# selftok-team/SelftokTokenizer

Hardware: AMD Instinct MI355X
Metric: images/sec encode+decode, 256x256 512-token (higher is better)
Workload: dtype f32

## Files before the change

include/selftok_hip.h:

```cpp
#ifndef SELFTOK_HIP_H
#define SELFTOK_HIP_H

#include <stddef.h>
#include <stdint.h>

#ifdef __cplusplus
extern "C" {
#endif

#ifndef __HIP__
typedef struct ihipStream_t* hipStream_t;
#endif

#define SELFTOK_OK 0
#define SELFTOK_EINVAL (-1)
#define SELFTOK_EHIP (-2)

#define SELFTOK_IDS_I32 1
#define SELFTOK_PRENORMED 2
#define SELFTOK_VQ_F16COARSE 8
#define SELFTOK_VQ_F16COARSE1 16
#define SELFTOK_VQ_RT(n) (((n) & 0xF) << 8)
#define SELFTOK_VQ_SPLIT(n) (((n) & 0xFF) << 16)

int selftok_version(void);
const char* selftok_last_error(void);

size_t selftok_vq_workspace_bytes(int N, int C);
int selftok_vq_encode_f32(const float* z, const float* codebook, void* ids, float* best, void* workspace,
                          int N, int C, int D, int flags, hipStream_t stream);
size_t selftok_vq_packed_bytes(int C, int D);
int selftok_vq_pack_codebook(const float* codebook, float* packed, int C, int D, hipStream_t stream);
int selftok_vq_encode_packed_f32(const float* z, const float* packed, void* ids, float* best, void* workspace,
                                 int N, int C, int D, int flags, hipStream_t stream);

int selftok_vq_argmax_partial_packed_f32(const float* z, const float* packed, void* workspace, int* nsplit_out,
                                         int N, int C, int D, int flags, hipStream_t stream);
int selftok_vq_finalize_packed(const void* workspace, const float* z, const float* packed, void* ids, float* best,
                               int N, int C, int D, int nsplit, int flags, hipStream_t stream);

int selftok_code_gather_ln_f32(const void* ids, const float* codebook, const float* ln_w, const float* ln_b,
                               float* out, int n, int C, int D, float eps, int flags, hipStream_t stream);

int selftok_vq_ema_accumulate_f32(const float* z, const void* ids, float* bins, float* embed_sum, int N, int C, int D, int flags, hipStream_t stream);
int selftok_vq_tpc_update_f32(float* tpc, const void* ids, int B, int K, int C, float weight, int flags, hipStream_t stream);
size_t selftok_vq_softmax_workspace_bytes(int N);
int selftok_vq_softmax_stats_f32(const float* z, const float* codebook, float* rowstats, float* colmean, void* workspace, int B, int K, int C, int D,
                                 float scale, int flags, hipStream_t stream);
int selftok_vq_softmax_backward_f32(const float* z, const float* codebook, const float* rowstats, const float* g_colmean, float* grad_z, void* workspace,
                                    int B, int K, int C, int D, float scale, int flags, hipStream_t stream);

int selftok_residual_ln_mod_f32(const float* x, const float* y, const float* gate, const float* shift, const float* scale,
                                float* x_out, float* n_out, int B, int T, int H,
                                long mod_stride_b, long mod_stride_t, long gate_stride_b, long gate_stride_t,
                                float eps, hipStream_t stream);
int selftok_residual_ln_mod_split(const float* x, const float* y, const float* gate, const float* shift, const float* scale,
                                  float* x_out, void* n_blk, int* overflow, int B, int T, int H,
                                  long mod_stride_b, long mod_stride_t, long gate_stride_b, long gate_stride_t,
                                  float eps, hipStream_t stream);

int selftok_bias_gelu_f32(float* h, const float* bias, long rows, int cols, hipStream_t stream);
int selftok_silu_f32(const float* in, float* out, long n, hipStream_t stream);
int selftok_add_rows_f32(const float* in, const float* table, float* out, int B, long per_sample, hipStream_t stream);
int selftok_timestep_embed_f32(const float* t, const float* freqs, float* out, int n, int dim, float t_scale, hipStream_t stream);
int selftok_patchify_f32(const float* x, float* out, int B, int C, int H, int W, hipStream_t stream);
int selftok_unpatchify_cfg_euler_f32(const float* y_cond, const float* y_uncond, const float* x, float* x_out, float* v_out,
                                     int B, int C, int hp, int wp, float dt, float cfg_scale, hipStream_t stream);
int selftok_rmsnorm_f32(const float* x, const float* w, float* out, long rows, int dim, float eps, hipStream_t stream);
int selftok_rotary_f32(const float* t, const float* freqs, float* out, long rows, int seq, int dim, float scale, hipStream_t stream);

#define SELFTOK_LINEAR_GELU 1
size_t selftok_linear_f16x2_packed_bytes(int N, int K);
int selftok_linear_f16x2_pack_weight(const float* W, void* packed, int N, int K, int* overflow, hipStream_t stream);
int selftok_linear_f16x2_f32(const float* A, long lda, const void* packed, const float* bias, float* out, long ldo,
                             int M, int N, int K, int flags, int* overflow, hipStream_t stream);
size_t selftok_split_f16x2_bytes(long rows, int cols);
int selftok_split_f16x2_f32(const float* x, long ld, void* blk, long rows, int cols, int* overflow, hipStream_t stream);
int selftok_linear_f16x2_split(const void* a_blk, const void* packed, const float* bias, float* out, void* out_blk, long ldo,
                               int M, int N, int K, int flags, int* overflow, hipStream_t stream);
int selftok_linear_f16x2_split_residual(const void* a_blk, const void* packed, const float* bias,
                                        const float* resid, long ldr, const float* gate, long gate_stride_b, long gate_stride_t, int T,
                                        float* out, long ldo, int M, int N, int K, int* overflow, hipStream_t stream);
size_t selftok_linear_f16x2_splitk_workspace_bytes(int M, int N, int ksplit);
int selftok_linear_f16x2_split_k(const void* a_blk, const void* packed, const float* bias, float* out, void* out_blk, long ldo,
                                 int M, int N, int K, int flags, int ksplit, void* workspace, int* overflow, hipStream_t stream);
int selftok_linear_f16x2_split_residual_k(const void* a_blk, const void* packed, const float* bias,
                                          const float* resid, long ldr, const float* gate, long gate_stride_b, long gate_stride_t, int T,
                                          float* out, long ldo, int M, int N, int K, int ksplit, void* workspace, int* overflow, hipStream_t stream);

#define SELFTOK_ATTN_F16X2 1
typedef struct selftok_attn_seg {
    const float* q; const float* k; const float* v; float* o;
    int len;
    long q_rs, k_rs, v_rs, o_rs;
    long q_bs, k_bs, v_bs, o_bs;
} selftok_attn_seg;
typedef struct selftok_attn_desc {
    selftok_attn_seg seg[2];
    int B, H, head_dim;
    const int* kvis;
    int seg0_sees_seg1;
    float scale;
    int mode;
    int* overflow;
    void* o_blk[2];
} selftok_attn_desc;
int selftok_attn_f32(const selftok_attn_desc* desc, hipStream_t stream);

int selftok_groupnorm_silu_bf16(const void* x, const void* weight, const void* bias, void* out, int B, int C, int HW, int groups,
                                float eps, int apply_silu, hipStream_t stream);
int selftok_latent_process_in(const void* moments_bf16, float* out, int B, int c_in, int c_keep, int HW, float shift, float scale, hipStream_t stream);
int selftok_latent_process_out(const float* z, void* out_bf16, long n, float shift, float scale, hipStream_t stream);
int selftok_clamp01_bf16(void* img, long n, hipStream_t stream);

size_t selftok_conv2d_packed_bytes(int Cout, int Cin, int ksize, int bn);
int selftok_conv2d_pack_weight_bf16(const void* w, void* packed, int Cout, int Cin, int ksize, int bn, hipStream_t stream);
int selftok_conv2d_nhwc_bf16(const void* x, const void* packed, const void* bias, const void* residual, void* out, int B, int H, int W, int Cin, int Cout,
                             int Cstore, int ldo, int ksize, int stride, int upsample, int bn, hipStream_t stream);
size_t selftok_groupnorm_nhwc_workspace_bytes(int B, int HW, int C);
int selftok_groupnorm_silu_nhwc_bf16(const void* x, const void* weight, const void* bias, void* out, void* workspace, int B, int HW, int C, int groups,
                                     float eps, int apply_silu, hipStream_t stream);

#define SELFTOK_VX_UPSAMPLE2X 8
int selftok_vx_conv2d_bf16(const void* x, const void* w, const void* bias, const void* residual, void* out, int B, int H, int W, int ldx, int Cin, int Cout,
                           int ksize, int stride, int order, hipStream_t stream);
size_t selftok_vx_groupnorm_workspace_bytes(int B, int HW, int C);
int selftok_vx_groupnorm_bf16(const void* x, const void* gamma, const void* beta, void* out, void* workspace, const void* silu_table, float* stats, int B, int HW,
                              int C, int groups, double eps, hipStream_t stream);
int selftok_vx_silu_table_bf16(void* table, hipStream_t stream);
size_t selftok_vx_attention_workspace_bytes(int B, int T, int C);
int selftok_vx_attention_bf16(const void* q, const void* k, const void* v, void* out, void* workspace, int B, int T, int C, hipStream_t stream);
int selftok_vx_expf_f32(const float* x, float* y, long n, hipStream_t stream);

#define SELFTOK_LINEAR_BIAS_LAST 2
#define SELFTOK_LINEAR_MKL_ORDER 4
#define SELFTOK_LINEAR_SPLIT(n) (((n) & 0xFF) << 8)
size_t selftok_linear_f32_workspace_bytes(long M, int N, int K, int flags);
int selftok_linear_f32(const float* x, long ldx, const float* w, const float* bias, const float* res, long ldr, int res_mod, const float* gate, long ldg,
                       int gate_mod, float* out, long ldo, long M, int N, int K, int flags, void* workspace, size_t workspace_bytes, hipStream_t stream);

#define SELFTOK_EX_GELU 1
#define SELFTOK_EX_BIAS_LAST 2
int selftok_ex_linear_f32(const float* x, long ldx, const float* w, const float* bias, const float* res, long ldr, int res_mod, const float* gate,
                          long ldg, int gate_mod, float* out, long ldo, long M, int N, int K, int gelu, hipStream_t stream);
int selftok_ex_layernorm_mod_f32(const float* x, long ldx, float* out, long ldo, const float* shift, const float* scale, long ldt, int T, const float* gamma,
                                 const float* beta, float* stats, long rows, int N, float eps, hipStream_t stream);
int selftok_ex_res_layernorm_mod_f32(const float* x, long ldx, const float* lin, long ldl, const float* lin_bias, const float* gate, long ldg, int gate_mod,
                                     float* x_out, long ldxo, float* out, long ldo, const float* shift, const float* scale, long ldt, int T, long rows, int N, float eps,
                                     hipStream_t stream);
int selftok_ex_unary_f32(const float* x, float* y, long n, int mode, hipStream_t stream);
size_t selftok_ex_attention_workspace_bytes(int B, int H, int Tq, int Tk, int D);
int selftok_ex_attention_f32(const float* q, long qs, const float* k1, const float* v1, long kvs1, int Tk1, int valid1, int rows1, const float* k2, const float* v2,
                             long kvs2, int Tk2, float* out, void* workspace, int B, int H, int Tq, int D, hipStream_t stream);
int selftok_ex_attention_fused_supported(int Tk1, int Tk2, int D);
int selftok_ex_attention_fused_f32(const float* q, long qs, const float* k1, const float* v1, long kvs1, int Tk1, int valid1, int rows1, const float* k2, const float* v2,
                                   long kvs2, int Tk2, float* out, int B, int H, int Tq, int D, hipStream_t stream);

#ifdef __cplusplus
}
#endif
#endif
```

selftoktokenizer_amd/csrc/attention.hip:

```cpp
#include "common.h"
#include "selftok_hip.h"
#include <stdlib.h>
#include <type_traits>

namespace selftok {

typedef float f32x16 __attribute__((ext_vector_type(16)));

struct AttnSeg {
    const float* q;
    const float* k;
    const float* v;
    float* o;
    _Float16* o_blk;
    int len;
    long q_rs, k_rs, v_rs, o_rs;
    long q_bs, k_bs, v_bs, o_bs;
};

struct AttnParams {
    AttnSeg seg[2];
    int B, H;
    const int* kvis;
    int seg0_sees_seg1;
    float scale;
    int qtiles;
    int xcd_remap;
    int prio;
};

constexpr int KT = 32;
constexpr int KSTR = 68;
constexpr int QROWS = 128;

__global__ __launch_bounds__(256) void attn64_kernel(AttnParams P)
{
    __shared__ __attribute__((aligned(16))) float s_kb[2][KT * KSTR];
    __shared__ __attribute__((aligned(16))) float s_vb[2][KT * 64];

    const int tid = threadIdx.x, lane = tid & 63, wave = tid >> 6;
    const int half = lane >> 5, col = lane & 31;
    int qt, h, b;
    {
        const int T = gridDim.x, orig = blockIdx.x;
        const int q8 = T >> 3, r8 = T & 7, xcd = orig & 7, idx = orig >> 3;
        const int w = P.xcd_remap ? (xcd < r8 ? xcd * (q8 + 1) : r8 * (q8 + 1) + (xcd - r8) * q8) + idx : orig;
        qt = w % P.qtiles;
        h = (w / P.qtiles) % P.H;
        b = w / (P.qtiles * P.H);
    }

    int n0 = P.seg[0].len;
    if (P.kvis) { int kv = P.kvis[b] + 1; n0 = kv < n0 ? (kv < 0 ? 0 : kv) : n0; }
    const int rows0 = P.seg[0].q ? n0 : 0;
    int s, r0;
    {
        const int t0 = P.seg[0].q ? (P.seg[0].len + QROWS - 1) / QROWS : 0;
        if (qt < t0) { s = 0; r0 = qt * QROWS; }
        else { s = 1; r0 = (qt - t0) * QROWS; }
    }
    const int rows_live = (s == 0) ? rows0 : (P.seg[1].q ? P.seg[1].len : 0);
    if (r0 >= rows_live) return;

    const AttnSeg& qs = P.seg[s];
    const int n1 = (s == 1 || P.seg0_sees_seg1) ? P.seg[1].len : 0;

    const int my_row = r0 + wave * 32 + col;
    const bool row_ok = my_row < rows_live;
    float qf[32];
    {
        const float* qp = qs.q + (size_t)b * qs.q_bs + (size_t)(row_ok ? my_row : (rows_live - 1)) * qs.q_rs + h * 64 + 32 * half;
#pragma unroll
        for (int j = 0; j < 8; ++j) {
            float4 t = *reinterpret_cast<const float4*>(qp + 4 * j);
            qf[4 * j] = t.x; qf[4 * j + 1] = t.y; qf[4 * j + 2] = t.z; qf[4 * j + 3] = t.w;
        }
    }

    f32x16 o0 = {0, 0, 0, 0, 0, 0, 0, 0, 0, 0, 0, 0, 0, 0, 0, 0};
    f32x16 o1 = o0;
    const float c = P.scale * 1.4426950408889634f;
    float m_run = -__builtin_inff(), l_run = 0.f;

    const int st_key = tid >> 4, st_part = tid & 15;
    float4 rk[2], rv[2];

    const float* kp = nullptr;
    const float* vp = nullptr;
    long k_step = 0, v_step = 0, k_half = 0, v_half = 0;
    auto set_segment = [&](int seg) {
        const AttnSeg& ks = P.seg[seg];
        kp = ks.k + (size_t)b * ks.k_bs + (size_t)st_key * ks.k_rs + h * 64 + st_part * 4;
        vp = ks.v + (size_t)b * ks.v_bs + (size_t)st_key * ks.v_rs + h * 64 + st_part * 4;
        k_step = (long)KT * ks.k_rs; v_step = (long)KT * ks.v_rs;
        k_half = 16 * ks.k_rs; v_half = 16 * ks.v_rs;
    };
    auto issue_loads = [&](int key0, int nkeys) {
#pragma unroll
        for (int u = 0; u < 2; ++u) {
            int key = key0 + st_key + 16 * u;
            if (key < nkeys) {
                rk[u] = *reinterpret_cast<const float4*>(kp + u * k_half);
                rv[u] = *reinterpret_cast<const float4*>(vp + u * v_half);
            } else {
                rk[u] = make_float4(0.f, 0.f, 0.f, 0.f);
                rv[u] = make_float4(0.f, 0.f, 0.f, 0.f);
            }
        }
        kp += k_step; vp += v_step;
    };

    const int nt0 = (n0 + KT - 1) / KT, nt1 = (n1 + KT - 1) / KT;
    const int ntiles = nt0 + nt1;
    if (ntiles == 0) return;
    set_segment(nt0 > 0 ? 0 : 1);
    issue_loads(0, nt0 > 0 ? n0 : n1);
    auto write_tile = [&](int buf) {
#pragma unroll
        for (int u = 0; u < 2; ++u) {
            int key = st_key + 16 * u;
            *reinterpret_cast<float4*>(&s_kb[buf][key * KSTR + st_part * 4]) = rk[u];
            *reinterpret_cast<float4*>(&s_vb[buf][key * 64 + st_part * 4]) = rv[u];
        }
    };
    write_tile(0);
    __syncthreads();

    for (int t = 0; t < ntiles; ++t) {
        const int seg = t < nt0 ? 0 : 1;
        const int key0 = (seg == 0 ? t : t - nt0) * KT;
        const int nkeys = seg == 0 ? n0 : n1;
        const float* s_k = s_kb[t & 1];
        const float* s_v = s_vb[t & 1];
        if (t + 1 < ntiles) {
            const int seg_n = (t + 1) < nt0 ? 0 : 1;
            if (t + 1 == nt0) set_segment(1);
            issue_loads((seg_n == 0 ? t + 1 : t + 1 - nt0) * KT, seg_n == 0 ? n0 : n1);
        }

        f32x16 sc = {0, 0, 0, 0, 0, 0, 0, 0, 0, 0, 0, 0, 0, 0, 0, 0};
#pragma unroll
        for (int j = 0; j < 8; ++j) {
            float4 kf = *reinterpret_cast<const float4*>(&s_k[col * KSTR + 32 * half + 4 * j]);
            sc = __builtin_amdgcn_mfma_f32_32x32x2f32(kf.x, qf[4 * j + 0], sc, 0, 0, 0);
            sc = __builtin_amdgcn_mfma_f32_32x32x2f32(kf.y, qf[4 * j + 1], sc, 0, 0, 0);
            sc = __builtin_amdgcn_mfma_f32_32x32x2f32(kf.z, qf[4 * j + 2], sc, 0, 0, 0);
            sc = __builtin_amdgcn_mfma_f32_32x32x2f32(kf.w, qf[4 * j + 3], sc, 0, 0, 0);
        }
        if (key0 + KT > nkeys) {
            asm volatile("; ragged tile");
#pragma unroll
            for (int r = 0; r < 16; ++r)
                if (key0 + (r & 3) + 8 * (r >> 2) + 4 * half >= nkeys) sc[r] = -__builtin_inff();
        }
        float mx;
        {
            float m0 = fmaxf(fmaxf(sc[0], sc[1]), sc[2]), m1 = fmaxf(fmaxf(sc[3], sc[4]), sc[5]);
            float m2 = fmaxf(fmaxf(sc[6], sc[7]), sc[8]), m3 = fmaxf(fmaxf(sc[9], sc[10]), sc[11]);
            float m4 = fmaxf(fmaxf(sc[12], sc[13]), sc[14]);
            mx = fmaxf(fmaxf(fmaxf(m0, m1), m2), fmaxf(fmaxf(m3, m4), sc[15]));
        }
        mx = fmaxf(mx, __shfl_xor(mx, 32, WAVE));
        const float m_new = fmaxf(m_run, mx * c);
        float psum = 0.f;
#pragma unroll
        for (int r = 0; r < 16; ++r) {
            float p = __builtin_amdgcn_exp2f(__builtin_fmaf(sc[r], c, -m_new));
            sc[r] = p;
            psum += p;
        }
        if (__any(m_new != m_run)) {
            const float alpha = __builtin_amdgcn_exp2f(m_run - m_new);
            l_run *= alpha;
#pragma unroll
            for (int r = 0; r < 16; ++r) { o0[r] *= alpha; o1[r] *= alpha; }
            m_run = m_new;
        }
        l_run += psum;

#pragma unroll
        for (int m = 0; m < 16; ++m) {
            const int key = (m & 3) + 8 * (m >> 2) + 4 * half;
            float v0 = s_v[key * 64 + col];
            float v1 = s_v[key * 64 + 32 + col];
            o0 = __builtin_amdgcn_mfma_f32_32x32x2f32(v0, sc[m], o0, 0, 0, 0);
            o1 = __builtin_amdgcn_mfma_f32_32x32x2f32(v1, sc[m], o1, 0, 0, 0);
        }
        if (t + 1 < ntiles) write_tile((t + 1) & 1);
        __syncthreads();
    }

    const float l_tot = l_run + __shfl_xor(l_run, 32, WAVE);
    const float inv = 1.0f / l_tot;
    if (row_ok) {
        float* op = qs.o + (size_t)b * qs.o_bs + (size_t)my_row * qs.o_rs + h * 64;
#pragma unroll
        for (int g = 0; g < 4; ++g) {
            const int d0 = 8 * g + 4 * half;
            *reinterpret_cast<float4*>(op + d0) = make_float4(o0[4 * g] * inv, o0[4 * g + 1] * inv, o0[4 * g + 2] * inv, o0[4 * g + 3] * inv);
            *reinterpret_cast<float4*>(op + 32 + d0) = make_float4(o1[4 * g] * inv, o1[4 * g + 1] * inv, o1[4 * g + 2] * inv, o1[4 * g + 3] * inv);
        }
    }
}

__device__ __forceinline__ void attn_lds_dma16(const void* base, unsigned voff, unsigned lds)
{
    asm volatile("s_mov_b32 m0, %2\n\ts_nop 0\n\tglobal_load_lds_dwordx4 %0, %1" ::"v"(voff), "s"(base), "s"(lds) : "memory", "m0");
}

__global__ __launch_bounds__(256) void attn64_dma_kernel(AttnParams P)
{
    __shared__ __attribute__((aligned(1024))) float s_kb[2][KT * 64];
    __shared__ __attribute__((aligned(1024))) float s_vb[2][KT * 64];

    const int tid = threadIdx.x, lane = tid & 63, wave = __builtin_amdgcn_readfirstlane(tid >> 6);
    const int half = lane >> 5, col = lane & 31;
    const bool prio = P.prio != 0;
    int qt, h, b;
    {
        const int T = gridDim.x, orig = blockIdx.x;
        const int q8 = T >> 3, r8 = T & 7, xcd = orig & 7, idx = orig >> 3;
        const int w = P.xcd_remap ? (xcd < r8 ? xcd * (q8 + 1) : r8 * (q8 + 1) + (xcd - r8) * q8) + idx : orig;
        qt = w % P.qtiles;
        h = (w / P.qtiles) % P.H;
        b = w / (P.qtiles * P.H);
    }
    int n0 = P.seg[0].len;
    if (P.kvis) { int kv = P.kvis[b] + 1; n0 = kv < n0 ? (kv < 0 ? 0 : kv) : n0; }
    const int rows0 = P.seg[0].q ? n0 : 0;
    int s, r0;
    {
        const int t0 = P.seg[0].q ? (P.seg[0].len + QROWS - 1) / QROWS : 0;
        if (qt < t0) { s = 0; r0 = qt * QROWS; }
        else { s = 1; r0 = (qt - t0) * QROWS; }
    }
    const int rows_live = (s == 0) ? rows0 : (P.seg[1].q ? P.seg[1].len : 0);
    if (r0 >= rows_live) return;
    const AttnSeg& qs = P.seg[s];
    const int n1 = (s == 1 || P.seg0_sees_seg1) ? P.seg[1].len : 0;

    const int my_row = r0 + wave * 32 + col;
    const bool row_ok = my_row < rows_live;
    float qf[32];
    {
        const float* qp = qs.q + (size_t)b * qs.q_bs + (size_t)(row_ok ? my_row : (rows_live - 1)) * qs.q_rs + h * 64 + 32 * half;
#pragma unroll
        for (int j = 0; j < 8; ++j) {
            float4 t = *reinterpret_cast<const float4*>(qp + 4 * j);
            qf[4 * j] = t.x; qf[4 * j + 1] = t.y; qf[4 * j + 2] = t.z; qf[4 * j + 3] = t.w;
        }
    }
    f32x16 o0 = {0, 0, 0, 0, 0, 0, 0, 0, 0, 0, 0, 0, 0, 0, 0, 0};
    f32x16 o1 = o0;
    const float c = P.scale * 1.4426950408889634f;
    float m_run = -__builtin_inff(), l_run = 0.f;

    const int kr = lane >> 4, pos = lane & 15;
    const int ksw = pos ^ ((4 * wave + kr) & 15);
    const unsigned lds_k = (unsigned)(size_t)(__attribute__((address_space(3))) float*)&s_kb[0][0];
    const unsigned lds_v = (unsigned)(size_t)(__attribute__((address_space(3))) float*)&s_vb[0][0];
    auto stage = [&](int seg, int key0, int nkeys, int buf) {
        const AttnSeg& ks = P.seg[seg];
        const char* kb = reinterpret_cast<const char*>(ks.k + (size_t)b * ks.k_bs + (size_t)key0 * ks.k_rs + h * 64);
        const char* vb = reinterpret_cast<const char*>(ks.v + (size_t)b * ks.v_bs + (size_t)key0 * ks.v_rs + h * 64);
        const unsigned krs = (unsigned)ks.k_rs * 4u, vrs = (unsigned)ks.v_rs * 4u;
        if (key0 + KT <= nkeys) {
            const unsigned ko = kr * krs + ksw * 16, vo = kr * vrs + pos * 16;
#pragma unroll
            for (int u = 0; u < 2; ++u) {
                const int i = wave + 4 * u;
                attn_lds_dma16(kb + (size_t)(4 * i) * krs, ko, lds_k + buf * (KT * 256) + i * 1024);
                attn_lds_dma16(vb + (size_t)(4 * i) * vrs, vo, lds_v + buf * (KT * 256) + i * 1024);
            }
        } else {
            const int last = nkeys - 1 - key0;
#pragma unroll
            for (int u = 0; u < 2; ++u) {
                const int i = wave + 4 * u;
                const int row = 4 * i + kr, src = row < last ? row : last;
                attn_lds_dma16(kb, (unsigned)src * krs + ksw * 16, lds_k + buf * (KT * 256) + i * 1024);
                attn_lds_dma16(vb, (unsigned)src * vrs + pos * 16, lds_v + buf * (KT * 256) + i * 1024);
            }
        }
    };
    int kaddr[8];
#pragma unroll
    for (int j = 0; j < 8; ++j) kaddr[j] = col * 64 + (((8 * half + j) ^ (col & 15)) << 2);

    const int nt0 = (n0 + KT - 1) / KT, nt1 = (n1 + KT - 1) / KT;
    const int ntiles = nt0 + nt1;
    if (ntiles == 0) return;
    stage(nt0 > 0 ? 0 : 1, 0, nt0 > 0 ? n0 : n1, 0);
    asm volatile("s_waitcnt vmcnt(0)" ::: "memory");
    __syncthreads();

    auto tile = [&](int t, auto BUF) {
        constexpr int buf = decltype(BUF)::value;
        const int seg = t < nt0 ? 0 : 1;
        const int key0 = (seg == 0 ? t : t - nt0) * KT;
        const int nkeys = seg == 0 ? n0 : n1;
        const float* s_k = s_kb[buf];
        const float* s_v = s_vb[buf];
        if (t + 1 < ntiles) {
            const int seg_n = (t + 1) < nt0 ? 0 : 1;
            stage(seg_n, (seg_n == 0 ? t + 1 : t + 1 - nt0) * KT, seg_n == 0 ? n0 : n1, buf ^ 1);
        }

        f32x16 sc = {0, 0, 0, 0, 0, 0, 0, 0, 0, 0, 0, 0, 0, 0, 0, 0};
        if (prio) __builtin_amdgcn_s_setprio(1);
#pragma unroll
        for (int j = 0; j < 8; ++j) {
            float4 kf = *reinterpret_cast<const float4*>(&s_k[kaddr[j]]);
            sc = __builtin_amdgcn_mfma_f32_32x32x2f32(kf.x, qf[4 * j + 0], sc, 0, 0, 0);
            sc = __builtin_amdgcn_mfma_f32_32x32x2f32(kf.y, qf[4 * j + 1], sc, 0, 0, 0);
            sc = __builtin_amdgcn_mfma_f32_32x32x2f32(kf.z, qf[4 * j + 2], sc, 0, 0, 0);
            sc = __builtin_amdgcn_mfma_f32_32x32x2f32(kf.w, qf[4 * j + 3], sc, 0, 0, 0);
        }
        if (prio) __builtin_amdgcn_s_setprio(0);
        if (key0 + KT > nkeys) {
            asm volatile("; ragged tile");
#pragma unroll
            for (int r = 0; r < 16; ++r)
                if (key0 + (r & 3) + 8 * (r >> 2) + 4 * half >= nkeys) sc[r] = -__builtin_inff();
        }
        float mx;
        {
            float m0 = fmaxf(fmaxf(sc[0], sc[1]), sc[2]), m1 = fmaxf(fmaxf(sc[3], sc[4]), sc[5]);
            float m2 = fmaxf(fmaxf(sc[6], sc[7]), sc[8]), m3 = fmaxf(fmaxf(sc[9], sc[10]), sc[11]);
            float m4 = fmaxf(fmaxf(sc[12], sc[13]), sc[14]);
            mx = fmaxf(fmaxf(fmaxf(m0, m1), m2), fmaxf(fmaxf(m3, m4), sc[15]));
        }
        mx = fmaxf(mx, __shfl_xor(mx, 32, WAVE));
        const float m_new = fmaxf(m_run, mx * c);
        float psum = 0.f;
#pragma unroll
        for (int r = 0; r < 16; ++r) {
            float p = __builtin_amdgcn_exp2f(__builtin_fmaf(sc[r], c, -m_new));
            sc[r] = p;
            psum += p;
        }
        if (__any(m_new != m_run)) {
            const float alpha = __builtin_amdgcn_exp2f(m_run - m_new);
            l_run *= alpha;
#pragma unroll
            for (int r = 0; r < 16; ++r) { o0[r] *= alpha; o1[r] *= alpha; }
            m_run = m_new;
        }
        l_run += psum;
        if (prio) __builtin_amdgcn_s_setprio(1);
#pragma unroll
        for (int m = 0; m < 16; ++m) {
            const int key = (m & 3) + 8 * (m >> 2) + 4 * half;
            float v0 = s_v[key * 64 + col];
            float v1 = s_v[key * 64 + 32 + col];
            o0 = __builtin_amdgcn_mfma_f32_32x32x2f32(v0, sc[m], o0, 0, 0, 0);
            o1 = __builtin_amdgcn_mfma_f32_32x32x2f32(v1, sc[m], o1, 0, 0, 0);
        }
        if (prio) __builtin_amdgcn_s_setprio(0);
        asm volatile("s_waitcnt vmcnt(0)" ::: "memory");
        __syncthreads();
    };
    for (int t = 0; t < ntiles; t += 2) {
        tile(t, std::integral_constant<int, 0>{});
        if (t + 1 < ntiles) tile(t + 1, std::integral_constant<int, 1>{});
    }

    const float l_tot = l_run + __shfl_xor(l_run, 32, WAVE);
    const float inv = 1.0f / l_tot;
    if (row_ok) {
        float* op = qs.o + (size_t)b * qs.o_bs + (size_t)my_row * qs.o_rs + h * 64;
#pragma unroll
        for (int g = 0; g < 4; ++g) {
            const int d0 = 8 * g + 4 * half;
            *reinterpret_cast<float4*>(op + d0) = make_float4(o0[4 * g] * inv, o0[4 * g + 1] * inv, o0[4 * g + 2] * inv, o0[4 * g + 3] * inv);
            *reinterpret_cast<float4*>(op + 32 + d0) = make_float4(o1[4 * g] * inv, o1[4 * g + 1] * inv, o1[4 * g + 2] * inv, o1[4 * g + 3] * inv);
        }
    }
}

typedef _Float16 h16x8 __attribute__((ext_vector_type(8)));
typedef unsigned u32x4 __attribute__((ext_vector_type(4)));
typedef unsigned u32x2 __attribute__((ext_vector_type(2)));

constexpr int KG_STRIDE = 32 * 16 + 16;
constexpr int K_PLANE = 8 * KG_STRIDE;
constexpr int V_PLANE = 4 * 64 * 16;
constexpr int KV_BUF = 2 * K_PLANE + 2 * V_PLANE;

typedef _Float16 h16x2 __attribute__((ext_vector_type(2)));
typedef float f32x2 __attribute__((ext_vector_type(2)));
struct HiLo { unsigned hi, lo; };
__device__ __forceinline__ HiLo split_pair(float a, float b)
{
    const f32x2 x = {a, b};
    const h16x2 h = __builtin_convertvector(x, h16x2);
    const h16x2 l = __builtin_convertvector(x - __builtin_convertvector(h, f32x2), h16x2);
    return HiLo{__builtin_bit_cast(unsigned, h), __builtin_bit_cast(unsigned, l)};
}
__device__ __forceinline__ HiLo split_pair_scaled(float a, float b)
{
    const f32x2 x = {a, b};
    const h16x2 h = __builtin_convertvector(x, h16x2);
    const h16x2 l = __builtin_convertvector((x - __builtin_convertvector(h, f32x2)) * 2048.0f, h16x2);
    return HiLo{__builtin_bit_cast(unsigned, h), __builtin_bit_cast(unsigned, l)};
}
__device__ __forceinline__ h16x8 as_h8(const u32x4& v) { return __builtin_bit_cast(h16x8, v); }
#if defined(SELFTOK_TUNE) && defined(SELFTOK_ATTN_PRESPLIT_PROBE)
__device__ __forceinline__ HiLo split_pair_kv(float a, float b)
{
    const f32x2 x = {a, b};
    return HiLo{__builtin_bit_cast(unsigned, __builtin_convertvector(x, h16x2)), 0u};
}
#else
__device__ __forceinline__ HiLo split_pair_kv(float a, float b) { return split_pair(a, b); }
#endif

__global__ __launch_bounds__(256, 2) void attn64_f16x2_kernel(AttnParams P, int* __restrict__ overflow)
{
    __shared__ __attribute__((aligned(16))) unsigned char s_kv[2 * KV_BUF];

    const int tid = threadIdx.x, lane = tid & 63, wave = tid >> 6;
    const int half = lane >> 5, col = lane & 31;
    int qt, h, b;
    {
        const int T = gridDim.x, orig = blockIdx.x;
        const int q8 = T >> 3, r8 = T & 7, xcd = orig & 7, idx = orig >> 3;
        const int w = (xcd < r8 ? xcd * (q8 + 1) : r8 * (q8 + 1) + (xcd - r8) * q8) + idx;
        qt = w % P.qtiles;
        h = (w / P.qtiles) % P.H;
        b = w / (P.qtiles * P.H);
    }
    int n0 = P.seg[0].len;
    if (P.kvis) { int kv = P.kvis[b] + 1; n0 = kv < n0 ? (kv < 0 ? 0 : kv) : n0; }
    const int rows0 = P.seg[0].q ? n0 : 0;
    int s, r0;
    {
        const int t0 = P.seg[0].q ? (P.seg[0].len + QROWS - 1) / QROWS : 0;
        if (qt < t0) { s = 0; r0 = qt * QROWS; }
        else { s = 1; r0 = (qt - t0) * QROWS; }
    }
    const int rows_live = (s == 0) ? rows0 : (P.seg[1].q ? P.seg[1].len : 0);
    if (r0 >= rows_live) return;
    const AttnSeg& qs = P.seg[s];
    const int n1 = (s == 1 || P.seg0_sees_seg1) ? P.seg[1].len : 0;

    const float c = P.scale * 1.4426950408889634f;
    const int my_row = r0 + wave * 32 + col;
    const bool row_ok = my_row < rows_live;
    u32x4 q0[4], q1[4];
    {
        const float* qp = qs.q + (size_t)b * qs.q_bs + (size_t)(row_ok ? my_row : (rows_live - 1)) * qs.q_rs + h * 64 + 8 * half;
#pragma unroll
        for (int ks = 0; ks < 4; ++ks) {
            const float4 a = *reinterpret_cast<const float4*>(qp + 16 * ks);
            const float4 c4 = *reinterpret_cast<const float4*>(qp + 16 * ks + 4);
            const float v[8] = {a.x * c, a.y * c, a.z * c, a.w * c, c4.x * c, c4.y * c, c4.z * c, c4.w * c};
#pragma unroll
            for (int j = 0; j < 4; ++j) { const HiLo t_ = split_pair(v[2 * j], v[2 * j + 1]); q0[ks][j] = t_.hi; q1[ks][j] = t_.lo; }
        }
    }

    f32x16 o0 = {0, 0, 0, 0, 0, 0, 0, 0, 0, 0, 0, 0, 0, 0, 0, 0};
    f32x16 o1 = o0;
    float m_run = -__builtin_inff(), l_run = 0.f;

    const bool is_k = tid < 128;
    const int u = tid & 127;
    const int st_key = is_k ? (u >> 2) : 4 * (u >> 4);
    const int st_d = is_k ? 16 * (u & 3) : 4 * (u & 15);
    float4 rg[4];
    const float* sp = nullptr;
    long s_rs = 0;
    auto set_segment = [&](int seg) {
        const AttnSeg& ks = P.seg[seg];
        if (is_k) { sp = ks.k + (size_t)b * ks.k_bs + (size_t)st_key * ks.k_rs + h * 64 + st_d; s_rs = ks.k_rs; }
        else { sp = ks.v + (size_t)b * ks.v_bs + (size_t)st_key * ks.v_rs + h * 64 + st_d; s_rs = ks.v_rs; }
    };
    auto issue_loads = [&](int key0, int nkeys) {
        if (is_k) {
            const bool ok = key0 + st_key < nkeys;
#pragma unroll
            for (int i = 0; i < 4; ++i) rg[i] = ok ? *reinterpret_cast<const float4*>(sp + 4 * i) : make_float4(0.f, 0.f, 0.f, 0.f);
        } else {
#pragma unroll
            for (int i = 0; i < 4; ++i)
                rg[i] = (key0 + st_key + i < nkeys) ? *reinterpret_cast<const float4*>(sp + i * s_rs) : make_float4(0.f, 0.f, 0.f, 0.f);
        }
        sp += (long)KT * s_rs;
    };
    auto write_tile = [&](int buf) {
        unsigned char* base = s_kv + buf * KV_BUF;
        if (is_k) {
            const float v[16] = {rg[0].x, rg[0].y, rg[0].z, rg[0].w, rg[1].x, rg[1].y, rg[1].z, rg[1].w,
                                 rg[2].x, rg[2].y, rg[2].z, rg[2].w, rg[3].x, rg[3].y, rg[3].z, rg[3].w};
#pragma unroll
            for (int e = 0; e < 2; ++e) {
                u32x4 hi, lo;
#pragma unroll
                for (int j = 0; j < 4; ++j) { const HiLo t_ = split_pair_kv(v[8 * e + 2 * j], v[8 * e + 2 * j + 1]); hi[j] = t_.hi; lo[j] = t_.lo; }
                const int g = (st_d >> 3) + e;
                *reinterpret_cast<u32x4*>(base + g * KG_STRIDE + st_key * 16) = hi;
                *reinterpret_cast<u32x4*>(base + K_PLANE + g * KG_STRIDE + st_key * 16) = lo;
            }
        } else {
            const float v[4][4] = {{rg[0].x, rg[0].y, rg[0].z, rg[0].w}, {rg[1].x, rg[1].y, rg[1].z, rg[1].w},
                                   {rg[2].x, rg[2].y, rg[2].z, rg[2].w}, {rg[3].x, rg[3].y, rg[3].z, rg[3].w}};
            const int kg = ((st_key >> 4) << 1) + ((st_key >> 2) & 1), hb = (st_key >> 3) & 1;
            unsigned char* vb = base + 2 * K_PLANE + kg * (64 * 16) + hb * 8;
#pragma unroll
            for (int i = 0; i < 4; ++i) {
                u32x2 hi, lo;
                { const HiLo t_ = split_pair_kv(v[0][i], v[1][i]); hi[0] = t_.hi; lo[0] = t_.lo; }
                { const HiLo t_ = split_pair_kv(v[2][i], v[3][i]); hi[1] = t_.hi; lo[1] = t_.lo; }
                const int dp = i * 16 + (st_d >> 2);
                *reinterpret_cast<u32x2*>(vb + dp * 16) = hi;
                *reinterpret_cast<u32x2*>(vb + V_PLANE + dp * 16) = lo;
            }
        }
    };

    const int nt0 = (n0 + KT - 1) / KT, nt1 = (n1 + KT - 1) / KT;
    const int ntiles = nt0 + nt1;
    if (ntiles == 0) return;
    set_segment(nt0 > 0 ? 0 : 1);
    issue_loads(0, nt0 > 0 ? n0 : n1);
    write_tile(0);
    __syncthreads();

    for (int t = 0; t < ntiles; ++t) {
        const int seg = t < nt0 ? 0 : 1;
        const int key0 = (seg == 0 ? t : t - nt0) * KT;
        const int nkeys = seg == 0 ? n0 : n1;
        const unsigned char* sb = s_kv + (t & 1) * KV_BUF;
        if (t + 1 < ntiles) {
            const int seg_n = (t + 1) < nt0 ? 0 : 1;
            if (t + 1 == nt0) set_segment(1);
            issue_loads((seg_n == 0 ? t + 1 : t + 1 - nt0) * KT, seg_n == 0 ? n0 : n1);
        }

        f32x16 sc = {0, 0, 0, 0, 0, 0, 0, 0, 0, 0, 0, 0, 0, 0, 0, 0};
#pragma unroll
        for (int ks = 0; ks < 4; ++ks) {
            const h16x8 k0 = *reinterpret_cast<const h16x8*>(sb + (2 * ks + half) * KG_STRIDE + col * 16);
            const h16x8 k1 = *reinterpret_cast<const h16x8*>(sb + K_PLANE + (2 * ks + half) * KG_STRIDE + col * 16);
            sc = __builtin_amdgcn_mfma_f32_32x32x16_f16(k0, as_h8(q0[ks]), sc, 0, 0, 0);
            sc = __builtin_amdgcn_mfma_f32_32x32x16_f16(k0, as_h8(q1[ks]), sc, 0, 0, 0);
            sc = __builtin_amdgcn_mfma_f32_32x32x16_f16(k1, as_h8(q0[ks]), sc, 0, 0, 0);
        }
        if (key0 + KT > nkeys) {
            asm volatile("; ragged tile");
#pragma unroll
            for (int r = 0; r < 16; ++r)
                if (key0 + (r & 3) + 8 * (r >> 2) + 4 * half >= nkeys) sc[r] = -__builtin_inff();
        }
        float mx;
        {
            float m0 = fmaxf(fmaxf(sc[0], sc[1]), sc[2]), m1 = fmaxf(fmaxf(sc[3], sc[4]), sc[5]);
            float m2 = fmaxf(fmaxf(sc[6], sc[7]), sc[8]), m3 = fmaxf(fmaxf(sc[9], sc[10]), sc[11]);
            float m4 = fmaxf(fmaxf(sc[12], sc[13]), sc[14]);
            mx = fmaxf(fmaxf(fmaxf(m0, m1), m2), fmaxf(fmaxf(m3, m4), sc[15]));
        }
        mx = fmaxf(mx, __shfl_xor(mx, 32, WAVE));
        const float m_new = fmaxf(m_run, mx);
        const f32x2 mm = {m_new, m_new};
        f32x2 psum = {0.f, 0.f};
        u32x4 p0[2], p1[2];
#pragma unroll
        for (int r = 0; r < 16; r += 2) {
            const f32x2 a = f32x2{sc[r], sc[r + 1]} - mm;
            const f32x2 p = {__builtin_amdgcn_exp2f(a[0]), __builtin_amdgcn_exp2f(a[1])};
            psum += p;
            { const HiLo t_ = split_pair(p[0], p[1]); p0[r >> 3][(r & 7) >> 1] = t_.hi; p1[r >> 3][(r & 7) >> 1] = t_.lo; }
        }
        if (__any(m_new != m_run)) {
            const float alpha = __builtin_amdgcn_exp2f(m_run - m_new);
            l_run *= alpha;
#pragma unroll
            for (int r = 0; r < 16; ++r) { o0[r] *= alpha; o1[r] *= alpha; }
            m_run = m_new;
        }
        l_run += psum[0] + psum[1];

#pragma unroll
        for (int ks2 = 0; ks2 < 2; ++ks2) {
            const unsigned char* vb = sb + 2 * K_PLANE + (2 * ks2 + half) * (64 * 16) + col * 16;
            const h16x8 va0 = *reinterpret_cast<const h16x8*>(vb), va1 = *reinterpret_cast<const h16x8*>(vb + V_PLANE);
            const h16x8 vb0 = *reinterpret_cast<const h16x8*>(vb + 32 * 16), vb1 = *reinterpret_cast<const h16x8*>(vb + V_PLANE + 32 * 16);
            o0 = __builtin_amdgcn_mfma_f32_32x32x16_f16(va0, as_h8(p0[ks2]), o0, 0, 0, 0);
            o1 = __builtin_amdgcn_mfma_f32_32x32x16_f16(vb0, as_h8(p0[ks2]), o1, 0, 0, 0);
            o0 = __builtin_amdgcn_mfma_f32_32x32x16_f16(va0, as_h8(p1[ks2]), o0, 0, 0, 0);
            o1 = __builtin_amdgcn_mfma_f32_32x32x16_f16(vb0, as_h8(p1[ks2]), o1, 0, 0, 0);
            o0 = __builtin_amdgcn_mfma_f32_32x32x16_f16(va1, as_h8(p0[ks2]), o0, 0, 0, 0);
            o1 = __builtin_amdgcn_mfma_f32_32x32x16_f16(vb1, as_h8(p0[ks2]), o1, 0, 0, 0);
        }
        if (t + 1 < ntiles) write_tile((t + 1) & 1);
        __syncthreads();
    }

    const float l_tot = l_run + __shfl_xor(l_run, 32, WAVE);
    const float inv = 1.0f / l_tot;
    float chk = l_tot * 0.f;
#pragma unroll
    for (int r = 0; r < 16; ++r) { chk = __builtin_fmaf(o0[r], 0.f, chk); chk = __builtin_fmaf(o1[r], 0.f, chk); }
    if (overflow && row_ok && chk != 0.f) atomicOr(overflow, 4);
    if (row_ok) {
        const size_t off = (size_t)b * qs.o_bs + (size_t)my_row * qs.o_rs + h * 64;
#pragma unroll
        for (int a = 0; a < 4; ++a)
#pragma unroll
            for (int bb = 0; bb < 2; ++bb) {
                const int r = a + 4 * bb;
                const int d = 4 * (a + 8 * bb + 4 * half);
                if (qs.o_blk) {
                    const HiLo ab = split_pair_scaled(opaque_f32(o0[r] * inv), opaque_f32(o0[r + 8] * inv));
                    const HiLo cd = split_pair_scaled(opaque_f32(o1[r] * inv), opaque_f32(o1[r + 8] * inv));
                    const long row_g = (long)b * qs.len + my_row;
                    *reinterpret_cast<uint2*>(qs.o_blk + split_blk_index(row_g, h * 64 + d, 0, P.H * 2)) = make_uint2(ab.hi, cd.hi);
                    *reinterpret_cast<uint2*>(qs.o_blk + split_blk_index(row_g, h * 64 + d, 1, P.H * 2)) = make_uint2(ab.lo, cd.lo);
                } else {
                    *reinterpret_cast<float4*>(qs.o + off + d) = make_float4(o0[r] * inv, o0[r + 8] * inv, o1[r] * inv, o1[r + 8] * inv);
                }
            }
    }
}

__global__ __launch_bounds__(256) void attn16_kernel(const float* __restrict__ q, const float* __restrict__ k, const float* __restrict__ v,
                                                     float* __restrict__ o, int L, long q_rs, long k_rs, long v_rs, long o_rs,
                                                     long q_bs, long k_bs, long v_bs, long o_bs, float scale)
{
    extern __shared__ __attribute__((aligned(16))) float smem[];
    float* s_k = smem;
    float* s_v = smem + (size_t)L * 16;
    const int b = blockIdx.y, h = blockIdx.x;
    for (int i = threadIdx.x; i < L * 4; i += blockDim.x) {
        int key = i >> 2, part = i & 3;
        *reinterpret_cast<float4*>(&s_k[key * 16 + part * 4]) = *reinterpret_cast<const float4*>(k + (size_t)b * k_bs + (size_t)key * k_rs + h * 16 + part * 4);
        *reinterpret_cast<float4*>(&s_v[key * 16 + part * 4]) = *reinterpret_cast<const float4*>(v + (size_t)b * v_bs + (size_t)key * v_rs + h * 16 + part * 4);
    }
    __syncthreads();
    const float c = scale * 1.4426950408889634f;
    for (int row = threadIdx.x; row < L; row += blockDim.x) {
        float qq[16], acc[16];
        const float* qp = q + (size_t)b * q_bs + (size_t)row * q_rs + h * 16;
#pragma unroll
        for (int j = 0; j < 4; ++j) {
            float4 t = *reinterpret_cast<const float4*>(qp + 4 * j);
            qq[4 * j] = t.x; qq[4 * j + 1] = t.y; qq[4 * j + 2] = t.z; qq[4 * j + 3] = t.w;
        }
#pragma unroll
        for (int d = 0; d < 16; ++d) acc[d] = 0.f;
        float m_run = -__builtin_inff(), l_run = 0.f;
        for (int key = 0; key < L; ++key) {
            float s = 0.f;
#pragma unroll
            for (int d = 0; d < 16; ++d) s = __builtin_fmaf(qq[d], s_k[key * 16 + d], s);
            float sl = s * c;
            float m_new = fmaxf(m_run, sl);
            float alpha = __builtin_amdgcn_exp2f(m_run - m_new);
            float p = __builtin_amdgcn_exp2f(sl - m_new);
            l_run = l_run * alpha + p;
#pragma unroll
            for (int d = 0; d < 16; ++d) acc[d] = __builtin_fmaf(p, s_v[key * 16 + d], acc[d] * alpha);
            m_run = m_new;
        }
        const float inv = 1.0f / l_run;
        float* op = o + (size_t)b * o_bs + (size_t)row * o_rs + h * 16;
#pragma unroll
        for (int j = 0; j < 4; ++j)
            *reinterpret_cast<float4*>(op + 4 * j) = make_float4(acc[4 * j] * inv, acc[4 * j + 1] * inv, acc[4 * j + 2] * inv, acc[4 * j + 3] * inv);
    }
}

}

using namespace selftok;

extern "C" {

int selftok_attn_f32(const selftok_attn_desc* d, hipStream_t stream)
{
    if (!d || d->B < 0 || d->H <= 0) { set_last_error("attn: bad descriptor"); return SELFTOK_EINVAL; }
    if (d->B == 0) return SELFTOK_OK;
    if (d->head_dim == 64) {
        AttnParams P;
        for (int s = 0; s < 2; ++s) {
            const selftok_attn_seg& a = d->seg[s];
            const bool osplit = d->mode == SELFTOK_ATTN_F16X2 && d->o_blk[s] != nullptr;
            if (d->o_blk[s] && (d->mode != SELFTOK_ATTN_F16X2 || ((size_t)d->o_blk[s] & 15))) { set_last_error("attn: split outputs need the f16x2 mode and 16-byte alignment"); return SELFTOK_EINVAL; }
            if (a.len < 0 || (a.len > 0 && (!a.k || !a.v)) || (a.q && !a.o && !osplit)) { set_last_error("attn: bad segment"); return SELFTOK_EINVAL; }
            if (((a.q_rs | a.k_rs | a.v_rs | a.o_rs | a.q_bs | a.k_bs | a.v_bs | a.o_bs) & 3) != 0) { set_last_error("attn: strides must be multiples of 4 floats"); return SELFTOK_EINVAL; }
            P.seg[s] = AttnSeg{a.len > 0 ? a.q : nullptr, a.k, a.v, a.o, (_Float16*)d->o_blk[s], a.len, a.q_rs, a.k_rs, a.v_rs, a.o_rs, a.q_bs, a.k_bs, a.v_bs, a.o_bs};
        }
        P.B = d->B; P.H = d->H; P.kvis = d->kvis; P.seg0_sees_seg1 = d->seg0_sees_seg1; P.scale = d->scale;
        int t0 = P.seg[0].q ? (P.seg[0].len + QROWS - 1) / QROWS : 0;
        int t1 = P.seg[1].q ? (P.seg[1].len + QROWS - 1) / QROWS : 0;
        if (t0 + t1 == 0) return SELFTOK_OK;
        P.qtiles = t0 + t1;
        P.xcd_remap = 1;
        P.prio = 0;
#ifdef SELFTOK_TUNE
        { const char* e = getenv("SELFTOK_ATTN_PRIO"); if (e) P.prio = atoi(e); }
#endif
        if (d->mode == SELFTOK_ATTN_F16X2) {
            hipLaunchKernelGGL(attn64_f16x2_kernel, dim3((t0 + t1) * d->H * d->B), dim3(256), 0, stream, P, d->overflow);
            return check_launch("attn64_f16x2_kernel");
        }
        if (d->mode != 0) { set_last_error("attn: unknown mode"); return SELFTOK_EINVAL; }
        bool dma = true;
        for (int s = 0; s < 2; ++s)
            if (P.seg[s].len > 0 && ((((size_t)P.seg[s].k | (size_t)P.seg[s].v) & 15) != 0 || P.seg[s].k_rs >= (1l << 24) || P.seg[s].v_rs >= (1l << 24))) dma = false;
#ifdef SELFTOK_TUNE
        { const char* e = getenv("SELFTOK_ATTN_VARIANT"); if (e && atoi(e) == 0) dma = false; }
#endif
        if (dma) {
            hipLaunchKernelGGL(attn64_dma_kernel, dim3((t0 + t1) * d->H * d->B), dim3(256), 0, stream, P);
            return check_launch("attn64_dma_kernel");
        }
        hipLaunchKernelGGL(attn64_kernel, dim3((t0 + t1) * d->H * d->B), dim3(256), 0, stream, P);
        return check_launch("attn64_kernel");
    }
    if (d->head_dim == 16) {
        const selftok_attn_seg& a = d->seg[1];
        if (d->seg[0].len != 0 || d->kvis || !a.q || !a.k || !a.v || !a.o || a.len <= 0 || a.len > 1024) { set_last_error("attn(head_dim 16): single unmasked segment of <= 1024 rows only"); return SELFTOK_EINVAL; }
        size_t lds = (size_t)a.len * 16 * 2 * sizeof(float);
        hipLaunchKernelGGL(attn16_kernel, dim3(d->H, d->B), dim3(256), lds, stream, a.q, a.k, a.v, a.o, a.len,
                           a.q_rs, a.k_rs, a.v_rs, a.o_rs, a.q_bs, a.k_bs, a.v_bs, a.o_bs, d->scale);
        return check_launch("attn16_kernel");
    }
    set_last_error("attn: head_dim must be 64 or 16");
    return SELFTOK_EINVAL;
}

}
```

Baseline: 3.200.

## Pack 32-row query units densely across waves and add deeper KV prefetch ring

Attention blocks now pack four independent 32-row query units, one per wave, instead of one 128-row tile per block. This cuts the idle waves that partially filled tiles and kvis-masked rows left behind, and a block's K/V staging covers the union of what its units need. The DMA kernel is templated on ring depth and group size so more tiles can be prefetched ahead with partial vmcnt waits; only a tuning build enables the deeper variants. A new F32_REG mode value is added, and waves without work still join every barrier, which adds some control overhead.

```diff
diff --git a/include/selftok_hip.h b/include/selftok_hip.h
--- a/include/selftok_hip.h
+++ b/include/selftok_hip.h
@@ -89,6 +89,7 @@
                                           float* out, long ldo, int M, int N, int K, int ksplit, void* workspace, int* overflow, hipStream_t stream);
 
 #define SELFTOK_ATTN_F16X2 1
+#define SELFTOK_ATTN_F32_REG 2
 typedef struct selftok_attn_seg {
     const float* q; const float* k; const float* v; float* o;
     int len;
diff --git a/selftoktokenizer_amd/csrc/attention.hip b/selftoktokenizer_amd/csrc/attention.hip
--- a/selftoktokenizer_amd/csrc/attention.hip
+++ b/selftoktokenizer_amd/csrc/attention.hip
@@ -203,15 +203,52 @@
     }
 }
 
+constexpr int UROWS = 32;
+
+struct PackedUnit {
+    int s;
+    int r0;
+    int rows_live;
+    int nt0, nt1;
+    int my_nt;
+    int n0, n1;
+};
+
+__device__ __forceinline__ bool packed_unit(const AttnParams& P, int qt, int b, int wave, PackedUnit& U)
+{
+    int n0 = P.seg[0].len;
+    if (P.kvis) { int kv = P.kvis[b] + 1; n0 = kv < n0 ? (kv < 0 ? 0 : kv) : n0; }
+    const int rows0 = P.seg[0].q ? n0 : 0;
+    const int rows1 = P.seg[1].q ? P.seg[1].len : 0;
+    const int u0 = (rows0 + UROWS - 1) / UROWS, total = u0 + (rows1 + UROWS - 1) / UROWS;
+    const int first = 4 * qt;
+    if (first >= total) return false;
+    const int last = first + 3 < total ? first + 3 : total - 1;
+    const int u = first + wave;
+    U.s = u >= u0 ? 1 : 0;
+    U.r0 = (U.s ? u - u0 : u) * UROWS;
+    U.rows_live = U.s ? rows1 : rows0;
+    U.n0 = n0;
+    U.n1 = (last >= u0 || P.seg0_sees_seg1) ? P.seg[1].len : 0;
+    U.nt0 = (n0 + KT - 1) / KT;
+    U.nt1 = (U.n1 + KT - 1) / KT;
+    U.my_nt = u < total ? U.nt0 + ((U.s == 1 || P.seg0_sees_seg1) ? U.nt1 : 0) : 0;
+    return U.nt0 + U.nt1 > 0;
+}
+
 __device__ __forceinline__ void attn_lds_dma16(const void* base, unsigned voff, unsigned lds)
 {
     asm volatile("s_mov_b32 m0, %2\n\ts_nop 0\n\tglobal_load_lds_dwordx4 %0, %1" ::"v"(voff), "s"(base), "s"(lds) : "memory", "m0");
 }
 
+template <int NST, int TPB>
 __global__ __launch_bounds__(256) void attn64_dma_kernel(AttnParams P)
 {
-    __shared__ __attribute__((aligned(1024))) float s_kb[2][KT * 64];
-    __shared__ __attribute__((aligned(1024))) float s_vb[2][KT * 64];
+    static_assert(NST % TPB == 0 && NST / TPB >= 2, "ring = whole groups, at least two");
+    constexpr int AHEAD = NST / TPB - 1;
+    constexpr int KEEP = 4 * TPB * (AHEAD - 1);
+    __shared__ __attribute__((aligned(1024))) float s_kb[NST][KT * 64];
+    __shared__ __attribute__((aligned(1024))) float s_vb[NST][KT * 64];
 
     const int tid = threadIdx.x, lane = tid & 63, wave = __builtin_amdgcn_readfirstlane(tid >> 6);
     const int half = lane >> 5, col = lane & 31;
@@ -225,24 +262,19 @@
         h = (w / P.qtiles) % P.H;
         b = w / (P.qtiles * P.H);
     }
-    int n0 = P.seg[0].len;
-    if (P.kvis) { int kv = P.kvis[b] + 1; n0 = kv < n0 ? (kv < 0 ? 0 : kv) : n0; }
-    const int rows0 = P.seg[0].q ? n0 : 0;
-    int s, r0;
-    {
-        const int t0 = P.seg[0].q ? (P.seg[0].len + QROWS - 1) / QROWS : 0;
-        if (qt < t0) { s = 0; r0 = qt * QROWS; }
-        else { s = 1; r0 = (qt - t0) * QROWS; }
-    }
-    const int rows_live = (s == 0) ? rows0 : (P.seg[1].q ? P.seg[1].len : 0);
-    if (r0 >= rows_live) return;
-    const AttnSeg& qs = P.seg[s];
-    const int n1 = (s == 1 || P.seg0_sees_seg1) ? P.seg[1].len : 0;
-
-    const int my_row = r0 + wave * 32 + col;
-    const bool row_ok = my_row < rows_live;
+    PackedUnit U;
+    if (!packed_unit(P, qt, b, wave, U)) return;
+    const AttnSeg& qs = P.seg[U.s];
+    const int n0 = U.n0, n1 = U.n1, nt0 = U.nt0, ntiles = U.nt0 + U.nt1;
+    const int my_nt = U.my_nt;
+    const int rows_live = U.rows_live;
+
+    const int my_row = U.r0 + col;
+    const bool row_ok = my_nt > 0 && my_row < rows_live;
     float qf[32];
-    {
+#pragma unroll
+    for (int j = 0; j < 32; ++j) qf[j] = 0.f;
+    if (my_nt > 0) {
         const float* qp = qs.q + (size_t)b * qs.q_bs + (size_t)(row_ok ? my_row : (rows_live - 1)) * qs.q_rs + h * 64 + 32 * half;
 #pragma unroll
         for (int j = 0; j < 8; ++j) {
@@ -283,16 +315,28 @@
             }
         }
     };
+    auto stage_tile = [&](int t, int buf) {
+        if (t < ntiles) {
+            const int seg = t < nt0 ? 0 : 1;
+            stage(seg, (seg == 0 ? t : t - nt0) * KT, seg == 0 ? n0 : n1, buf);
+        }
+    };
+    auto close_group = [&](bool steady) {
+        if constexpr (AHEAD == 1) {
+            asm volatile("s_waitcnt vmcnt(0)" ::: "memory");
+            __syncthreads();
+        } else {
+            if (steady) asm volatile("s_waitcnt vmcnt(%0) lgkmcnt(0)\n\ts_barrier" ::"n"(KEEP) : "memory");
+            else asm volatile("s_waitcnt vmcnt(0) lgkmcnt(0)\n\ts_barrier" ::: "memory");
+        }
+    };
     int kaddr[8];
 #pragma unroll
     for (int j = 0; j < 8; ++j) kaddr[j] = col * 64 + (((8 * half + j) ^ (col & 15)) << 2);
 
-    const int nt0 = (n0 + KT - 1) / KT, nt1 = (n1 + KT - 1) / KT;
-    const int ntiles = nt0 + nt1;
-    if (ntiles == 0) return;
-    stage(nt0 > 0 ? 0 : 1, 0, nt0 > 0 ? n0 : n1, 0);
-    asm volatile("s_waitcnt vmcnt(0)" ::: "memory");
-    __syncthreads();
+#pragma unroll
+    for (int i = 0; i < AHEAD * TPB; ++i) stage_tile(i, i);
+    close_group(AHEAD * TPB <= ntiles);
 
     auto tile = [&](int t, auto BUF) {
         constexpr int buf = decltype(BUF)::value;
@@ -301,11 +345,12 @@
         const int nkeys = seg == 0 ? n0 : n1;
         const float* s_k = s_kb[buf];
         const float* s_v = s_vb[buf];
-        if (t + 1 < ntiles) {
-            const int seg_n = (t + 1) < nt0 ? 0 : 1;
-            stage(seg_n, (seg_n == 0 ? t + 1 : t + 1 - nt0) * KT, seg_n == 0 ? n0 : n1, buf ^ 1);
-        }
-
+        if constexpr (buf % TPB == 0) {
+#pragma unroll
+            for (int i = 0; i < TPB; ++i) stage_tile(t + AHEAD * TPB + i, (buf + AHEAD * TPB + i) % NST);
+        }
+
+        if (t < my_nt) {
         f32x16 sc = {0, 0, 0, 0, 0, 0, 0, 0, 0, 0, 0, 0, 0, 0, 0, 0};
         if (prio) __builtin_amdgcn_s_setprio(1);
 #pragma unroll
@@ -357,12 +402,14 @@
             o1 = __builtin_amdgcn_mfma_f32_32x32x2f32(v1, sc[m], o1, 0, 0, 0);
         }
         if (prio) __builtin_amdgcn_s_setprio(0);
-        asm volatile("s_waitcnt vmcnt(0)" ::: "memory");
-        __syncthreads();
-    };
-    for (int t = 0; t < ntiles; t += 2) {
+        }
+        if (buf % TPB == TPB - 1 || t + 1 >= ntiles) close_group((t / TPB + AHEAD + 1) * TPB <= ntiles);
+    };
+    for (int t = 0; t < ntiles; t += NST) {
         tile(t, std::integral_constant<int, 0>{});
         if (t + 1 < ntiles) tile(t + 1, std::integral_constant<int, 1>{});
+        if constexpr (NST > 2) { if (t + 2 < ntiles) tile(t + 2, std::integral_constant<int, 2>{}); }
+        if constexpr (NST > 3) { if (t + 3 < ntiles) tile(t + 3, std::integral_constant<int, 3>{}); }
     }
 
     const float l_tot = l_run + __shfl_xor(l_run, 32, WAVE);
@@ -419,7 +466,7 @@
 {
     __shared__ __attribute__((aligned(16))) unsigned char s_kv[2 * KV_BUF];
 
-    const int tid = threadIdx.x, lane = tid & 63, wave = tid >> 6;
+    const int tid = threadIdx.x, lane = tid & 63, wave = __builtin_amdgcn_readfirstlane(tid >> 6);
     const int half = lane >> 5, col = lane & 31;
     int qt, h, b;
     {
@@ -430,25 +477,20 @@
         h = (w / P.qtiles) % P.H;
         b = w / (P.qtiles * P.H);
     }
-    int n0 = P.seg[0].len;
-    if (P.kvis) { int kv = P.kvis[b] + 1; n0 = kv < n0 ? (kv < 0 ? 0 : kv) : n0; }
-    const int rows0 = P.seg[0].q ? n0 : 0;
-    int s, r0;
-    {
-        const int t0 = P.seg[0].q ? (P.seg[0].len + QROWS - 1) / QROWS : 0;
-        if (qt < t0) { s = 0; r0 = qt * QROWS; }
-        else { s = 1; r0 = (qt - t0) * QROWS; }
-    }
-    const int rows_live = (s == 0) ? rows0 : (P.seg[1].q ? P.seg[1].len : 0);
-    if (r0 >= rows_live) return;
-    const AttnSeg& qs = P.seg[s];
-    const int n1 = (s == 1 || P.seg0_sees_seg1) ? P.seg[1].len : 0;
+    PackedUnit U;
+    if (!packed_unit(P, qt, b, wave, U)) return;
+    const AttnSeg& qs = P.seg[U.s];
+    const int n0 = U.n0, n1 = U.n1;
+    const int my_nt = U.my_nt;
+    const int rows_live = U.rows_live;
 
     const float c = P.scale * 1.4426950408889634f;
-    const int my_row = r0 + wave * 32 + col;
-    const bool row_ok = my_row < rows_live;
+    const int my_row = U.r0 + col;
+    const bool row_ok = my_nt > 0 && my_row < rows_live;
     u32x4 q0[4], q1[4];
-    {
+#pragma unroll
+    for (int ks = 0; ks < 4; ++ks) { q0[ks] = u32x4{0, 0, 0, 0}; q1[ks] = u32x4{0, 0, 0, 0}; }
+    if (my_nt > 0) {
         const float* qp = qs.q + (size_t)b * qs.q_bs + (size_t)(row_ok ? my_row : (rows_live - 1)) * qs.q_rs + h * 64 + 8 * half;
 #pragma unroll
         for (int ks = 0; ks < 4; ++ks) {
@@ -519,9 +561,8 @@
         }
     };
 
-    const int nt0 = (n0 + KT - 1) / KT, nt1 = (n1 + KT - 1) / KT;
-    const int ntiles = nt0 + nt1;
-    if (ntiles == 0) return;
+    const int nt0 = U.nt0;
+    const int ntiles = U.nt0 + U.nt1;
     set_segment(nt0 > 0 ? 0 : 1);
     issue_loads(0, nt0 > 0 ? n0 : n1);
     write_tile(0);
@@ -538,6 +579,7 @@
             issue_loads((seg_n == 0 ? t + 1 : t + 1 - nt0) * KT, seg_n == 0 ? n0 : n1);
         }
 
+        if (t < my_nt) {
         f32x16 sc = {0, 0, 0, 0, 0, 0, 0, 0, 0, 0, 0, 0, 0, 0, 0, 0};
 #pragma unroll
         for (int ks = 0; ks < 4; ++ks) {
@@ -592,6 +634,7 @@
             o1 = __builtin_amdgcn_mfma_f32_32x32x16_f16(vb0, as_h8(p1[ks2]), o1, 0, 0, 0);
             o0 = __builtin_amdgcn_mfma_f32_32x32x16_f16(va1, as_h8(p0[ks2]), o0, 0, 0, 0);
             o1 = __builtin_amdgcn_mfma_f32_32x32x16_f16(vb1, as_h8(p0[ks2]), o1, 0, 0, 0);
+        }
         }
         if (t + 1 < ntiles) write_tile((t + 1) & 1);
         __syncthreads();
@@ -692,30 +735,39 @@
             P.seg[s] = AttnSeg{a.len > 0 ? a.q : nullptr, a.k, a.v, a.o, (_Float16*)d->o_blk[s], a.len, a.q_rs, a.k_rs, a.v_rs, a.o_rs, a.q_bs, a.k_bs, a.v_bs, a.o_bs};
         }
         P.B = d->B; P.H = d->H; P.kvis = d->kvis; P.seg0_sees_seg1 = d->seg0_sees_seg1; P.scale = d->scale;
-        int t0 = P.seg[0].q ? (P.seg[0].len + QROWS - 1) / QROWS : 0;
-        int t1 = P.seg[1].q ? (P.seg[1].len + QROWS - 1) / QROWS : 0;
+        const int t0 = P.seg[0].q ? (P.seg[0].len + QROWS - 1) / QROWS : 0;
+        const int t1 = P.seg[1].q ? (P.seg[1].len + QROWS - 1) / QROWS : 0;
         if (t0 + t1 == 0) return SELFTOK_OK;
-        P.qtiles = t0 + t1;
+        const int units = (P.seg[0].q ? (P.seg[0].len + UROWS - 1) / UROWS : 0) + (P.seg[1].q ? (P.seg[1].len + UROWS - 1) / UROWS : 0);
+        P.qtiles = (units + 3) / 4;
         P.xcd_remap = 1;
         P.prio = 0;
 #ifdef SELFTOK_TUNE
         { const char* e = getenv("SELFTOK_ATTN_PRIO"); if (e) P.prio = atoi(e); }
 #endif
         if (d->mode == SELFTOK_ATTN_F16X2) {
-            hipLaunchKernelGGL(attn64_f16x2_kernel, dim3((t0 + t1) * d->H * d->B), dim3(256), 0, stream, P, d->overflow);
+            hipLaunchKernelGGL(attn64_f16x2_kernel, dim3(P.qtiles * d->H * d->B), dim3(256), 0, stream, P, d->overflow);
             return check_launch("attn64_f16x2_kernel");
         }
-        if (d->mode != 0) { set_last_error("attn: unknown mode"); return SELFTOK_EINVAL; }
-        bool dma = true;
+        if (d->mode != 0 && d->mode != SELFTOK_ATTN_F32_REG) { set_last_error("attn: unknown mode"); return SELFTOK_EINVAL; }
+        bool dma = d->mode == 0;
         for (int s = 0; s < 2; ++s)
             if (P.seg[s].len > 0 && ((((size_t)P.seg[s].k | (size_t)P.seg[s].v) & 15) != 0 || P.seg[s].k_rs >= (1l << 24) || P.seg[s].v_rs >= (1l << 24))) dma = false;
+        int variant = 1;
 #ifdef SELFTOK_TUNE
-        { const char* e = getenv("SELFTOK_ATTN_VARIANT"); if (e && atoi(e) == 0) dma = false; }
+        { const char* e = getenv("SELFTOK_ATTN_VARIANT"); if (e) variant = atoi(e); if (variant == 0) dma = false; }
 #endif
         if (dma) {
-            hipLaunchKernelGGL(attn64_dma_kernel, dim3((t0 + t1) * d->H * d->B), dim3(256), 0, stream, P);
+            const dim3 grid(P.qtiles * d->H * d->B);
+#ifdef SELFTOK_TUNE
+            if (variant == 3) { hipLaunchKernelGGL((attn64_dma_kernel<3, 1>), grid, dim3(256), 0, stream, P); return check_launch("attn64_dma_kernel<3,1>"); }
+            if (variant == 4) { hipLaunchKernelGGL((attn64_dma_kernel<4, 2>), grid, dim3(256), 0, stream, P); return check_launch("attn64_dma_kernel<4,2>"); }
+#endif
+            (void)variant;
+            hipLaunchKernelGGL((attn64_dma_kernel<2, 1>), grid, dim3(256), 0, stream, P);
             return check_launch("attn64_dma_kernel");
         }
+        P.qtiles = t0 + t1;
         hipLaunchKernelGGL(attn64_kernel, dim3((t0 + t1) * d->H * d->B), dim3(256), 0, stream, P);
         return check_launch("attn64_kernel");
     }
```

Measured after the change: 3.202, median of 6. About the same (+0.1%).
